# aidilayce/FollowMyHold

Hardware: AMD Instinct MI355X
Metric: guidance-steps/sec (512x512, 778+20k verts) (higher is better)
Workload: dtype f32; 1 GPU; configs[1]: 512x512 frame/GPU, 778-vert hand + 10242-vert/20480-face object, joint step (phase C); images_per_gpu=1, global_images=1, parallelism=image-sharded x1, steps_per_graph=1

## Files before the change

### followmyhold_amd/csrc/k_flexi.inc

```
#include "flexi_core.h"

constexpr int FX_ITEMS = 2048;

struct FlexiWs {
    uint8_t* cse;
    int32_t *npatch, *v_off, *ecross, *f_off, *bsum_v, *bsum_f;
    size_t total;
};
static FlexiWs carve_flexi(void* ws, int res) {
    const size_t G = (size_t)res + 1, C = (size_t)res * res * res, E = 3 * G * G * G;
    const size_t nbv = (C + FX_ITEMS - 1) / FX_ITEMS, nbf = (E + FX_ITEMS - 1) / FX_ITEMS;
    char* p = (char*)ws;
    Carve cv;
    FlexiWs w;
    w.cse = (uint8_t*)(p + cv.take(C));
    w.npatch = (int32_t*)(p + cv.take(C * 4));
    w.v_off = (int32_t*)(p + cv.take(C * 4));
    w.ecross = (int32_t*)(p + cv.take(E * 4));
    w.f_off = (int32_t*)(p + cv.take(E * 4));
    w.bsum_v = (int32_t*)(p + cv.take((nbv + 1) * 4));
    w.bsum_f = (int32_t*)(p + cv.take((nbf + 1) * 4));
    w.total = cv.off;
    return w;
}

extern "C" size_t foho_flexi_workspace_bytes(int32_t res) {
    if (res < 1 || res > 1024) return 0;
    return carve_flexi(nullptr, res).total;
}

__global__ __launch_bounds__(256) void k_flexi_classify(const float* s, int res, uint8_t* cse, int32_t* npatch, int32_t* ecross) {
    const int G = res + 1;
    const size_t t = (size_t)blockIdx.x * 256 + threadIdx.x;
    const size_t C = (size_t)res * res * res, G3 = (size_t)G * G * G;
    if (t < C) {
        const int k = (int)(t % res), j = (int)((t / res) % res), i = (int)(t / ((size_t)res * res));
        const unsigned code = flexi_cube_code(s, res, i, j, k);
        cse[t] = (uint8_t)code;
        npatch[t] = c_flexi_npatch[code];
    }
    if (t < 3 * G3) {
        const int axis = (int)(t / G3);
        const size_t r = t % G3;
        const int k = (int)(r % G), j = (int)((r / G) % G), i = (int)(r / ((size_t)G * G));
        const int di = axis == 0, dj = axis == 1, dk = axis == 2;
        int flag = 0;
        const bool along = (di ? i : (dj ? j : k)) < res;
        const bool t1 = di ? (j >= 1 && j <= res - 1) : (i >= 1 && i <= res - 1);
        const bool t2 = dk ? (j >= 1 && j <= res - 1) : (k >= 1 && k <= res - 1);
        if (along && t1 && t2) {
            const float sa = s[r], sb = s[((size_t)(i + di) * G + (j + dj)) * G + (k + dk)];
            flag = ((sa < 0.0f) != (sb < 0.0f)) ? 1 : 0;
        }
        ecross[t] = flag;
    }
}

__global__ __launch_bounds__(256) void k_scan_sums(const int32_t* in, size_t n, int32_t* bsum) {
    __shared__ int s_w[4];
    const size_t base = (size_t)blockIdx.x * FX_ITEMS + (size_t)threadIdx.x * 8;
    int v = 0;
#pragma unroll
    for (int q = 0; q < 8; q++) v += (base + q < n) ? in[base + q] : 0;
    const unsigned w = wave_sum((unsigned)v);
    if (lane_id() == 0) s_w[wave_id()] = (int)w;
    __syncthreads();
    if (threadIdx.x == 0) bsum[blockIdx.x] = (s_w[0] + s_w[1]) + (s_w[2] + s_w[3]);
}
__global__ __launch_bounds__(256) void k_scan_bsums(int32_t* bsum, int nb, int32_t* total) {
    __shared__ int s_w[4];
    __shared__ int s_carry;
    if (threadIdx.x == 0) s_carry = 0;
    __syncthreads();
    for (int base = 0; base < nb; base += 256) {
        const int i = base + threadIdx.x;
        const int v = (i < nb) ? bsum[i] : 0;
        const unsigned incl = wave_incl_scan((unsigned)v);
        if (lane_id() == 63) s_w[wave_id()] = (int)incl;
        __syncthreads();
        int off = s_carry;
        for (int w = 0; w < wave_id(); w++) off += s_w[w];
        if (i < nb) bsum[i] = off + (int)incl - v;
        __syncthreads();
        if (threadIdx.x == 0) s_carry += (s_w[0] + s_w[1]) + (s_w[2] + s_w[3]);
        __syncthreads();
    }
    if (threadIdx.x == 0) {
        bsum[nb] = s_carry;
        *total = s_carry;
    }
}
__global__ __launch_bounds__(256) void k_scan_apply(const int32_t* in, size_t n, const int32_t* bsum, int32_t* out) {
    __shared__ int s_w[4];
    const size_t base = (size_t)blockIdx.x * FX_ITEMS + (size_t)threadIdx.x * 8;
    int v[8], sum = 0;
#pragma unroll
    for (int q = 0; q < 8; q++) {
        v[q] = (base + q < n) ? in[base + q] : 0;
        sum += v[q];
    }
    const unsigned incl = wave_incl_scan((unsigned)sum);
    if (lane_id() == 63) s_w[wave_id()] = (int)incl;
    __syncthreads();
    int off = bsum[blockIdx.x] + (int)incl - sum;
    for (int w = 0; w < wave_id(); w++) off += s_w[w];
#pragma unroll
    for (int q = 0; q < 8; q++) {
        if (base + q < n) out[base + q] = off;
        off += v[q];
    }
}

struct Scan2 {
    const int32_t* in[2];
    size_t n[2];
    int32_t* bsum[2];
    int32_t* out[2];
    int nb[2];
};
__global__ __launch_bounds__(256) void k_scan2_sums(Scan2 a) {
    __shared__ int s_w[4];
    const int which = ((int)blockIdx.x < a.nb[0]) ? 0 : 1;
    const int blk = which ? blockIdx.x - a.nb[0] : blockIdx.x;
    const int32_t* in = which ? a.in[1] : a.in[0];
    const size_t n = which ? a.n[1] : a.n[0];
    const size_t base = (size_t)blk * FX_ITEMS + (size_t)threadIdx.x * 8;
    int v = 0;
#pragma unroll
    for (int q = 0; q < 8; q++) v += (base + q < n) ? in[base + q] : 0;
    const unsigned w = wave_sum((unsigned)v);
    if (lane_id() == 0) s_w[wave_id()] = (int)w;
    __syncthreads();
    if (threadIdx.x == 0) (which ? a.bsum[1] : a.bsum[0])[blk] = (s_w[0] + s_w[1]) + (s_w[2] + s_w[3]);
}
__device__ __forceinline__ int block_prefix(const int32_t* bsum, int blk, int* s_w) {
    int v = 0;
    for (int i = threadIdx.x; i < blk; i += 256) v += bsum[i];
    const unsigned w = wave_sum((unsigned)v);
    __syncthreads();
    if (lane_id() == 0) s_w[wave_id()] = (int)w;
    __syncthreads();
    const int r = (s_w[0] + s_w[1]) + (s_w[2] + s_w[3]);
    __syncthreads();
    return r;
}
__global__ __launch_bounds__(256) void k_scan2_apply(Scan2 a, int32_t* counts) {
    __shared__ int s_w[4];
    const int which = ((int)blockIdx.x < a.nb[0]) ? 0 : 1;
    const int blk = which ? blockIdx.x - a.nb[0] : blockIdx.x;
    const int32_t* in = which ? a.in[1] : a.in[0];
    const int32_t* bsum = which ? a.bsum[1] : a.bsum[0];
    int32_t* out = which ? a.out[1] : a.out[0];
    const size_t n = which ? a.n[1] : a.n[0];
    const size_t base = (size_t)blk * FX_ITEMS + (size_t)threadIdx.x * 8;
    int v[8], sum = 0;
#pragma unroll
    for (int q = 0; q < 8; q++) {
        v[q] = (base + q < n) ? in[base + q] : 0;
        sum += v[q];
    }
    const int prefix = block_prefix(bsum, blk, s_w);
    const unsigned incl = wave_incl_scan((unsigned)sum);
    if (lane_id() == 63) s_w[wave_id()] = (int)incl;
    __syncthreads();
    int off = prefix + (int)incl - sum;
    for (int w = 0; w < wave_id(); w++) off += s_w[w];
#pragma unroll
    for (int q = 0; q < 8; q++) {
        if (base + q < n) out[base + q] = off;
        off += v[q];
    }
    if (counts && blk == (which ? a.nb[1] : a.nb[0]) - 1 && threadIdx.x == 255) {
        if (which == 0) {
            counts[0] = off;
            counts[2] = 0;
        } else {
            counts[1] = 2 * off;
        }
    }
}
__global__ __launch_bounds__(256) void k_scan_apply_p(const int32_t* in, size_t n, const int32_t* bsum, int32_t* out) {
    __shared__ int s_w[4];
    const size_t base = (size_t)blockIdx.x * FX_ITEMS + (size_t)threadIdx.x * 8;
    int v[8], sum = 0;
#pragma unroll
    for (int q = 0; q < 8; q++) {
        v[q] = (base + q < n) ? in[base + q] : 0;
        sum += v[q];
    }
    const int prefix = block_prefix(bsum, (int)blockIdx.x, s_w);
    const unsigned incl = wave_incl_scan((unsigned)sum);
    if (lane_id() == 63) s_w[wave_id()] = (int)incl;
    __syncthreads();
    int off = prefix + (int)incl - sum;
    for (int w = 0; w < wave_id(); w++) off += s_w[w];
#pragma unroll
    for (int q = 0; q < 8; q++) {
        if (base + q < n) out[base + q] = off;
        off += v[q];
    }
}

__device__ __forceinline__ void flexi_corners(const float* x, const float* s, int res, size_t t, float* sc, float* xc) {
    const int G = res + 1;
    const int k = (int)(t % res), j = (int)((t / res) % res), i = (int)(t / ((size_t)res * res));
#pragma unroll
    for (int c = 0; c < 8; c++) {
        const size_t gi = ((size_t)(i + (c & 1)) * G + (j + ((c >> 1) & 1))) * G + (k + (c >> 2));
        sc[c] = s[gi];
        for (int q = 0; q < 3; q++) xc[3 * c + q] = x[3 * gi + q];
    }
}

__device__ __forceinline__ void flexi_verts_role(size_t t, const float* x, const float* s, int res, const uint8_t* cse, const int32_t* npatch,
                                                 const int32_t* v_off, float* verts, float* ldev, int cap, int32_t* counts) {
    if (t >= (size_t)res * res * res) return;
    const int np = npatch[t];
    if (np == 0) return;
    const int base = v_off[t];
    if (base + np > cap) {
        atomicOr(&counts[2], 1);
        return;
    }
    const unsigned code = cse[t];
    float sc[8], xc[24];
    flexi_corners(x, s, res, t, sc, xc);
    for (int p = 0; p < np; p++) flexi_dual_vertex(code, p, sc, xc, verts + 3 * (size_t)(base + p), ldev ? ldev + (base + p) : nullptr);
}

__device__ __forceinline__ void flexi_faces_role(size_t t, const float* s, int res, const uint8_t* cse, const int32_t* v_off,
                                                 const int32_t* ecross, const int32_t* f_off, int64_t* faces, int cap, int32_t* counts) {
    const int G = res + 1;
    const size_t G3 = (size_t)G * G * G;
    if (t >= 3 * G3 || !ecross[t]) return;
    const int qd = f_off[t];
    if (2 * qd + 2 > cap) {
        atomicOr(&counts[2], 2);
        return;
    }
    const int axis = (int)(t / G3);
    const size_t r = t % G3;
    const int k = (int)(r % G), j = (int)((r / G) % G), i = (int)(r / ((size_t)G * G));
    int64_t q[4];
#pragma unroll
    for (int c = 0; c < 4; c++) {
        const int ci = i + c_flexi_ring[axis][c][0], cj = j + c_flexi_ring[axis][c][1], ck = k + c_flexi_ring[axis][c][2];
        const size_t cid = ((size_t)ci * res + cj) * res + ck;
        q[c] = (int64_t)v_off[cid] + c_flexi_edge_patch[cse[cid]][c_flexi_ring[axis][c][3]];
    }
    flexi_quad(q, s[r] < 0.0f, faces + 6 * (size_t)qd);
}

__global__ __launch_bounds__(256) void k_flexi_emit(const float* x, const float* s, int res, const uint8_t* cse, const int32_t* npatch,
                                                    const int32_t* v_off, const int32_t* ecross, const int32_t* f_off, float* verts,
                                                    float* ldev, int verts_cap, int64_t* faces, int faces_cap, int32_t* counts, int nvb) {
    if ((int)blockIdx.x < nvb)
        flexi_verts_role((size_t)blockIdx.x * 256 + threadIdx.x, x, s, res, cse, npatch, v_off, verts, ldev, verts_cap, counts);
    else
        flexi_faces_role((size_t)(blockIdx.x - nvb) * 256 + threadIdx.x, s, res, cse, v_off, ecross, f_off, faces, faces_cap, counts);
}

extern "C" int foho_flexi_fwd(const float* x, const float* s, int32_t res, float* verts, int32_t verts_cap, int64_t* faces,
                              int32_t faces_cap, float* l_dev, int32_t* counts, void* workspace, size_t workspace_bytes,
                              void* stream_) {
    if (!x || !s || !verts || !faces || !counts || res < 1 || res > 1024 || verts_cap < 0 || faces_cap < 0) {
        foho_set_error("foho_flexi_fwd: bad argument");
        return FOHO_ERR_BAD_ARG;
    }
    const FlexiWs w = carve_flexi(workspace, res);
    if (!workspace || workspace_bytes < w.total) {
        foho_set_error("foho_flexi_fwd: workspace too small (query foho_flexi_workspace_bytes)");
        return FOHO_ERR_WORKSPACE;
    }
    hipStream_t stream = (hipStream_t)stream_;
    const size_t G = (size_t)res + 1, C = (size_t)res * res * res, E = 3 * G * G * G;
    const int nbv = (int)((C + FX_ITEMS - 1) / FX_ITEMS), nbf = (int)((E + FX_ITEMS - 1) / FX_ITEMS);
    hipLaunchKernelGGL(k_flexi_classify, dim3((unsigned)((E + 255) / 256)), dim3(256), 0, stream, s, res, w.cse, w.npatch, w.ecross);
    CHECK_LAUNCH("k_flexi_classify");
    Scan2 sc;
    sc.in[0] = w.npatch, sc.in[1] = w.ecross;
    sc.n[0] = C, sc.n[1] = E;
    sc.bsum[0] = w.bsum_v, sc.bsum[1] = w.bsum_f;
    sc.out[0] = w.v_off, sc.out[1] = w.f_off;
    sc.nb[0] = nbv, sc.nb[1] = nbf;
    hipLaunchKernelGGL(k_scan2_sums, dim3(nbv + nbf), dim3(256), 0, stream, sc);
    CHECK_LAUNCH("k_scan2_sums");
    hipLaunchKernelGGL(k_scan2_apply, dim3(nbv + nbf), dim3(256), 0, stream, sc, counts);
    CHECK_LAUNCH("k_scan2_apply");
    const int nvb = (int)((C + 255) / 256);
    hipLaunchKernelGGL(k_flexi_emit, dim3((unsigned)(nvb + (E + 255) / 256)), dim3(256), 0, stream, x, s, res, w.cse, w.npatch, w.v_off,
                       w.ecross, w.f_off, verts, l_dev, verts_cap, faces, faces_cap, counts, nvb);
    CHECK_LAUNCH("k_flexi_emit");
    return FOHO_OK;
}

__global__ __launch_bounds__(256) void k_flexi_bwd(const float* x, const float* s, int res, const uint8_t* cse, const int32_t* npatch,
                                                   const int32_t* v_off, const float* gverts, int n_verts, float* gs, float* gx) {
    const size_t t = (size_t)blockIdx.x * 256 + threadIdx.x;
    if (t >= (size_t)res * res * res) return;
    const int np = npatch[t];
    if (np == 0) return;
    const int base = v_off[t];
    if (base + np > n_verts) return;
    const int G = res + 1;
    const int k = (int)(t % res), j = (int)((t / res) % res), i = (int)(t / ((size_t)res * res));
    FLEXI_EDGE_TABLES
    const unsigned code = cse[t];
    float sc[8], xc[24];
    flexi_corners(x, s, res, t, sc, xc);
    for (int p = 0; p < np; p++) {
        float cnt = 0.f;
#pragma unroll
        for (int e = 0; e < 12; e++) cnt += (c_flexi_edge_patch[code][e] == p) ? 1.0f : 0.0f;
        float g[3];
        for (int q = 0; q < 3; q++) g[q] = gverts[3 * (size_t)(base + p) + q] / cnt;
#pragma unroll
        for (int e = 0; e < 12; e++) {
            if (c_flexi_edge_patch[code][e] != p) continue;
            const int a = fx_ea[e], b = fx_eb[e];
            const size_t ga = ((size_t)(i + (a & 1)) * G + (j + ((a >> 1) & 1))) * G + (k + (a >> 2));
            const size_t gb = ((size_t)(i + (b & 1)) * G + (j + ((b >> 1) & 1))) * G + (k + (b >> 2));
            const float D = sc[b] - sc[a];
            float dot = 0.f;
            for (int q = 0; q < 3; q++) dot += g[q] * (xc[3 * a + q] - xc[3 * b + q]);
            const float wa = sc[b] / D, wb = -sc[a] / D;
            atomicAdd(&gs[ga], dot * (wa / D));
            atomicAdd(&gs[gb], dot * (wb / D));
            if (gx) {
                for (int q = 0; q < 3; q++) {
                    atomicAdd(&gx[3 * ga + q], g[q] * wa);
                    atomicAdd(&gx[3 * gb + q], g[q] * wb);
                }
            }
        }
    }
}

extern "C" int foho_flexi_bwd(const float* x, const float* s, int32_t res, const float* grad_verts, int32_t n_verts, float* grad_s,
                              float* grad_x, const void* workspace, size_t workspace_bytes, void* stream_) {
    if (!x || !s || !grad_verts || !grad_s || res < 1 || res > 1024 || n_verts < 0) {
        foho_set_error("foho_flexi_bwd: bad argument");
        return FOHO_ERR_BAD_ARG;
    }
    const FlexiWs w = carve_flexi(const_cast<void*>(workspace), res);
    if (!workspace || workspace_bytes < w.total) {
        foho_set_error("foho_flexi_bwd: workspace too small");
        return FOHO_ERR_WORKSPACE;
    }
    hipStream_t stream = (hipStream_t)stream_;
    const size_t C = (size_t)res * res * res;
    hipLaunchKernelGGL(k_flexi_bwd, dim3((unsigned)((C + 255) / 256)), dim3(256), 0, stream, x, s, res, w.cse, w.npatch, w.v_off, grad_verts,
                       n_verts, grad_s, grad_x);
    CHECK_LAUNCH("k_flexi_bwd");
    return FOHO_OK;
}
```

### followmyhold_amd/csrc/k_object.inc

```

__global__ __launch_bounds__(256) void k_object_adopt(Ctx c, foho_image* img_rw, int32_t* faces_rw, const int32_t* counts,
                                                      const int64_t* obj_faces, int verts_cap, int faces_cap, int32_t* cnt) {
    const int b = blockIdx.y;
    const int v_off = img_rw[b].v_off, Vh = img_rw[b].Vh, f_off = img_rw[b].f_off, Fh = img_rw[b].Fh;
    int nv = counts[3 * b], nf = counts[3 * b + 1];
    const bool over = counts[3 * b + 2] != 0 || nv < 0 || nf < 0 || nv > verts_cap || nf > faces_cap;
    const bool odd = !over && (nf & 1);
    const bool bad = over || odd;
    if (bad) nv = nf = 0;
    const int64_t* src = obj_faces + (size_t)b * faces_cap * 3;
    int32_t* dst = faces_rw + 3 * (size_t)(f_off + Fh);
    const int shift = v_off + Vh;
    for (int j = blockIdx.x * 256 + threadIdx.x; j < 3 * nf; j += gridDim.x * 256) {
        const int v = (int32_t)src[j] + shift;
        dst[j] = v;
        atomicAdd(&cnt[v], 1);
    }
    const int32_t* hf = faces_rw + 3 * (size_t)f_off;
    for (int j = blockIdx.x * 256 + threadIdx.x; j < 3 * Fh; j += gridDim.x * 256) atomicAdd(&cnt[hf[j]], 1);
    if (blockIdx.x == 0 && threadIdx.x == 0) {
        img_rw[b].Vo = nv;
        img_rw[b].Fo = nf;
        img_rw[b].n_edges = 3 * nf / 2;
        if (bad) atomicOr(&c.flags[b], over ? 16 : 32);
        else if (nv == 0 || nf == 0) atomicOr(&c.flags[b], 64);
        for (int m = 0; m < 2; m++)
            for (int a = 0; a < 3; a++) c.mesh_info[2 * b + m].kmin_inv[a] = c.mesh_info[2 * b + m].kmax[a] = 0ull;
    }
}

__global__ __launch_bounds__(256) void k_object_fill(Ctx c, BboxCfg bc, int fgrid, const int32_t* inc_off, int32_t* cursor,
                                                     int32_t* inc_tmp) {
    if ((int)blockIdx.x >= fgrid) return bbox_role(c, bc, (int)blockIdx.x - fgrid, (int)blockIdx.y);
    const foho_image im = c.img[blockIdx.y];
    const int t = blockIdx.x * 256 + threadIdx.x;
    if (t >= 3 * (im.Fh + im.Fo)) return;
    const int v = c.faces[3 * (size_t)im.f_off + t], face = im.f_off + t / 3, corner = t % 3;
    inc_tmp[inc_off[v] + atomicAdd(&cursor[v], 1)] = (face << 2) | corner;
}

constexpr int TOPO_LDS_STRIDE = TOPO_MAXVAL + 1;
constexpr int TOPO_FAST = 16;
__global__ __launch_bounds__(64) void k_topo_finish_b(const int32_t* faces, int Vtot, int Fkey, const uint8_t* obj_flag,
                                                      const int32_t* inc_off, const int32_t* inc_tmp, int32_t* inc_fc,
                                                      int32_t* nbr_idx, unsigned long long* pair_v, const foho_image* img, int B, int32_t* flags,
                                                      int32_t* cnt, int32_t* cursor) {
    __shared__ int s_e[64 * TOPO_LDS_STRIDE], s_d[64 * TOPO_LDS_STRIDE], s_p[64 * TOPO_LDS_STRIDE];
    const int v = blockIdx.x * 64 + threadIdx.x;
    if (v >= Vtot) return;
    const int e0 = inc_off[v], n = inc_off[v + 1] - e0;
    cnt[v] = 0;
    cursor[v] = 0;
    if (n <= 0) return;
    int bad = 0;
    if (n > TOPO_MAXVAL) {
        bad = 1;
    } else if (n <= TOPO_FAST) {
        int x[TOPO_FAST], f[TOPO_FAST][3];
#pragma unroll
        for (int u = 0; u < TOPO_FAST; u++) x[u] = inc_tmp[e0 + min(u, n - 1)];
#pragma unroll
        for (int u = 0; u < TOPO_FAST; u++)
            for (int k = 0; k < 3; k++) f[u][k] = faces[3 * (size_t)(x[u] >> 2) + k];
        unsigned key[TOPO_FAST];
        int d[TOPO_FAST], pv[TOPO_FAST];
#pragma unroll
        for (int u = 0; u < TOPO_FAST; u++) {
            const int corner = x[u] & 3;
            key[u] = (u < n) ? (((unsigned)corner << 28) | (unsigned)(x[u] >> 2)) : 0xffffffffu;
            d[u] = (u < n) ? ((corner == 0) ? f[u][1] : ((corner == 1) ? f[u][2] : f[u][0])) : 0x7fffffff;
            pv[u] = (corner == 0) ? f[u][2] : ((corner == 1) ? f[u][0] : f[u][1]);
        }
        const bool check = obj_flag[v] != 0;
#pragma unroll
        for (int u = 0; u < TOPO_FAST; u++) {
            int rk = 0, rd = 0, dup = 0, found = 0;
#pragma unroll
            for (int j = 0; j < TOPO_FAST; j++) {
                rk += (key[j] < key[u]) ? 1 : 0;
                rd += (d[j] < d[u] || (d[j] == d[u] && j < u)) ? 1 : 0;
                dup |= (j < u && d[j] == d[u]) ? 1 : 0;
                found |= (d[j] == pv[u]) ? 1 : 0;
            }
            if (u < n) {
                inc_fc[e0 + rk] = x[u];
                pair_v[e0 + rk] = pack_pair(f[u][0], f[u][1], f[u][2], x[u] & 3);
                nbr_idx[e0 + rd] = d[u];
                if (check) bad |= dup | (found ^ 1);
            }
        }
    } else {
        int* e = s_e + threadIdx.x * TOPO_LDS_STRIDE;
        int* d = s_d + threadIdx.x * TOPO_LDS_STRIDE;
        int* pv = s_p + threadIdx.x * TOPO_LDS_STRIDE;
        for (int base = 0; base < n; base += 8) {
            int x[8];
#pragma unroll
            for (int u = 0; u < 8; u++) x[u] = inc_tmp[e0 + min(base + u, n - 1)];
#pragma unroll
            for (int u = 0; u < 8; u++)
                if (base + u < n) e[base + u] = x[u];
        }
        for (int a = 1; a < n; a++) {
            const int x = e[a];
            const long long kx = (long long)(x & 3) * Fkey + (x >> 2);
            int b2 = a - 1;
            while (b2 >= 0) {
                const int y = e[b2];
                if (((long long)(y & 3) * Fkey + (y >> 2)) <= kx) break;
                e[b2 + 1] = y;
                b2--;
            }
            e[b2 + 1] = x;
        }
        for (int base = 0; base < n; base += 8) {
            int x[8], f[8][3];
#pragma unroll
            for (int u = 0; u < 8; u++) x[u] = e[min(base + u, n - 1)];
#pragma unroll
            for (int u = 0; u < 8; u++)
                for (int k = 0; k < 3; k++) f[u][k] = faces[3 * (size_t)(x[u] >> 2) + k];
#pragma unroll
            for (int u = 0; u < 8; u++) {
                if (base + u >= n) break;
                const int corner = x[u] & 3;
                inc_fc[e0 + base + u] = x[u];
                pair_v[e0 + base + u] = pack_pair(f[u][0], f[u][1], f[u][2], corner);
                d[base + u] = (corner == 0) ? f[u][1] : ((corner == 1) ? f[u][2] : f[u][0]);
                pv[base + u] = (corner == 0) ? f[u][2] : ((corner == 1) ? f[u][0] : f[u][1]);
            }
        }
        for (int a = 1; a < n; a++) {
            const int x = d[a];
            int b2 = a - 1;
            while (b2 >= 0) {
                const int y = d[b2];
                if (y <= x) break;
                d[b2 + 1] = y;
                b2--;
            }
            d[b2 + 1] = x;
        }
        for (int q = 0; q < n; q++) nbr_idx[e0 + q] = d[q];
        if (obj_flag[v]) {
            for (int q = 1; q < n; q++) bad |= (d[q] == d[q - 1]);
            for (int q = 0; q < n && !bad; q++) {
                const int p = pv[q];
                bool found = false;
                for (int r = 0; r < n; r++) found = found || (d[r] == p);
                bad = !found;
            }
        }
    }
    if (bad)
        for (int b = 0; b < B; b++)
            if (v >= img[b].v_off && v < img[b].v_off + img[b].Vh + img[b].Vo) atomicOr(&flags[b], 32);
}

extern "C" size_t foho_object_workspace_bytes(int32_t Vtot, int32_t Ftot) {
    if (Vtot < 1 || Ftot < 1) return 0;
    const size_t n = (size_t)Vtot + 1, nb = (n + FX_ITEMS - 1) / FX_ITEMS;
    return 2 * al(n * 4) + al((nb + 1) * 4) + al((size_t)Ftot * 3 * 4);
}

extern "C" int foho_object_update(const foho_step_desc* desc, const int32_t* counts, const int64_t* obj_faces,
                                  int32_t faces_cap, const uint8_t* obj_flag, void* workspace, size_t workspace_bytes,
                                  void* stream_) {
    if (!desc || !counts || !obj_faces || !obj_flag || faces_cap < 0) {
        foho_set_error("foho_object_update: null argument");
        return FOHO_ERR_BAD_ARG;
    }
    const foho_dims& d = desc->dims;
    if (d.B < 1 || d.Vtot < 1 || d.Ftot < 1 || d.Ftot >= (1 << 28) || d.Fmax < 1 || faces_cap > d.Fo_max) {
        foho_set_error("foho_object_update: bad dims (Vo_max / Fo_max are the per-image object capacities)");
        return FOHO_ERR_BAD_ARG;
    }
    if (!pair_limits_ok(d)) {
        foho_set_error("foho_object_update: more than 4194304 vertex slots per batch or 524287 per image is not supported (pair table)");
        return FOHO_ERR_BAD_ARG;
    }
    const WS w = make_ws(d);
    if (!desc->workspace || desc->workspace_bytes < w.total || !workspace ||
        workspace_bytes < foho_object_workspace_bytes(d.Vtot, d.Ftot)) {
        foho_set_error("foho_object_update: workspace too small (foho_step_workspace_bytes / foho_object_workspace_bytes)");
        return FOHO_ERR_WORKSPACE;
    }
    hipStream_t stream = (hipStream_t)stream_;
    Ctx c = make_ctx(*desc, w);
    const size_t n = (size_t)d.Vtot + 1;
    const int nb = (int)((n + FX_ITEMS - 1) / FX_ITEMS);
    char* p = (char*)workspace;
    int32_t* cnt = (int32_t*)p;
    int32_t* cursor = (int32_t*)(p + al(n * 4));
    int32_t* bsum = (int32_t*)(p + 2 * al(n * 4));
    int32_t* inc_tmp = (int32_t*)(p + 2 * al(n * 4) + al(((size_t)nb + 1) * 4));
    const int fgrid = cdiv(3 * d.Fmax, 256);
    hipLaunchKernelGGL(k_object_adopt, dim3(std::max(1, std::min(fgrid, 128)), d.B), dim3(256), 0, stream, c,
                       const_cast<foho_image*>(desc->images), const_cast<int32_t*>(desc->faces), counts, obj_faces, d.Vo_max, faces_cap, cnt);
    CHECK_LAUNCH("k_object_adopt");
    hipLaunchKernelGGL(k_scan_sums, dim3(nb), dim3(256), 0, stream, cnt, n, bsum);
    CHECK_LAUNCH("k_scan_sums");
    hipLaunchKernelGGL(k_scan_apply_p, dim3(nb), dim3(256), 0, stream, cnt, n, bsum, const_cast<int32_t*>(desc->inc_off));
    CHECK_LAUNCH("k_scan_apply_p");
    BboxCfg bc;
    bc.nbh = cdiv(d.Vh_max > 0 ? d.Vh_max : 1, 256);
    bc.nbo = cdiv(d.Vo_max > 0 ? d.Vo_max : 1, 256);
    hipLaunchKernelGGL(k_object_fill, dim3(fgrid + bc.nbh + bc.nbo, d.B), dim3(256), 0, stream, c, bc, fgrid, desc->inc_off, cursor, inc_tmp);
    CHECK_LAUNCH("k_object_fill");
    hipLaunchKernelGGL(k_topo_finish_b, dim3(cdiv(d.Vtot, 64)), dim3(64), 0, stream, desc->faces, d.Vtot, d.Ftot, obj_flag, desc->inc_off,
                       inc_tmp, const_cast<int32_t*>(desc->inc_fc), const_cast<int32_t*>(desc->nbr_idx), c.pair_v, desc->images, d.B,
                       desc->flags, cnt, cursor);
    CHECK_LAUNCH("k_topo_finish_b");
    return FOHO_OK;
}
```

### followmyhold_amd/csrc/k_vertex.inc

```

__device__ __forceinline__ void load_moge(const Ctx& c, const foho_image& im, int mesh, int gi, float* v) {
    const float x = c.verts_in[3 * gi], y = c.verts_in[3 * gi + 1], z = c.verts_in[3 * gi + 2];
    if (mesh == 0) {
        v[0] = x;
        v[1] = y;
        v[2] = z;
    } else {
        const float* M = im.T_h2m;
        v[0] = ((x * M[0] + y * M[1]) + z * M[2]) + M[3];
        v[1] = ((x * M[4] + y * M[5]) + z * M[6]) + M[7];
        v[2] = ((x * M[8] + y * M[9]) + z * M[10]) + M[11];
    }
}

struct BboxCfg {
    int nbh, nbo;
};
__global__ __launch_bounds__(64) void k_bbox_clear(MeshInfo* mi, int n) {
    const int i = blockIdx.x * 64 + threadIdx.x;
    if (i < n)
        for (int a = 0; a < 3; a++) mi[i].kmin_inv[a] = mi[i].kmax[a] = 0ull;
}
__device__ void bbox_role(const Ctx& c, const BboxCfg& cfg, int bx, int b) {
    __shared__ unsigned long long s_k[6][4];
    const foho_image im = c.img[b];
    const int mesh = (bx < cfg.nbh) ? 0 : 1;
    const int blk = mesh ? (bx - cfg.nbh) : bx;
    const int n = mesh ? im.Vo : im.Vh;
    if (blk * 256 >= n) return;
    const int base = im.v_off + (mesh ? im.Vh : 0);
    const int i = blk * 256 + threadIdx.x;
    unsigned long long k[6] = {0ull, 0ull, 0ull, 0ull, 0ull, 0ull};
    if (i < n) {
        float v[3];
        load_moge(c, im, mesh, base + i, v);
        for (int a = 0; a < 3; a++) {
            const unsigned long long o = (unsigned long long)f2ord(v[a]) << 32;
            k[a] = ~(o | (unsigned)i);
            k[3 + a] = o | (unsigned)(~(unsigned)i);
        }
    }
    for (int a = 0; a < 6; a++) {
        unsigned long long x = k[a];
#pragma unroll
        for (int o = 32; o > 0; o >>= 1) {
            const unsigned long long y = __shfl_down(x, o, 64);
            x = (y > x) ? y : x;
        }
        if (lane_id() == 0) s_k[a][wave_id()] = x;
    }
    __syncthreads();
    if (threadIdx.x < 6) {
        unsigned long long x = s_k[threadIdx.x][0];
        for (int w = 1; w < 4; w++) x = (s_k[threadIdx.x][w] > x) ? s_k[threadIdx.x][w] : x;
        MeshInfo* mi = &c.mesh_info[b * 2 + mesh];
        unsigned long long* dst = (threadIdx.x < 3) ? &mi->kmin_inv[threadIdx.x] : &mi->kmax[threadIdx.x - 3];
        atomicMax(dst, x);
    }
}
__global__ __launch_bounds__(256) void k_bbox(Ctx c, BboxCfg cfg) { bbox_role(c, cfg, (int)blockIdx.x, (int)blockIdx.y); }

__global__ __launch_bounds__(256) void k_pair_table(Ctx c, int n) {
    const int e = blockIdx.x * 256 + threadIdx.x;
    if (e >= n) return;
    const int fc = c.inc_fc[e], f = fc >> 2;
    c.pair_v[e] = pack_pair(c.faces[3 * f], c.faces[3 * f + 1], c.faces[3 * f + 2], fc & 3);
}

__device__ void world_boxes(const Ctx& c, const foho_image& im, int b, float* s_box) {
    if (wave_id() == 0) {
        float v[12];
        for (int mesh = 0; mesh < 2; mesh++) {
            for (int a = 0; a < 3; a++) {
                v[6 * mesh + a] = INFINITY;
                v[6 * mesh + 3 + a] = -INFINITY;
            }
            const int nb = ((mesh ? im.Vo : im.Vh) + 255) / 256;
            for (int blk = lane_id(); blk < nb; blk += 64) {
                const float* row = c.xf_part + (((size_t)b * 2 + mesh) * VERT_BLOCKS_MAX + blk) * 8;
                for (int a = 0; a < 3; a++) {
                    v[6 * mesh + a] = fminf(v[6 * mesh + a], row[a]);
                    v[6 * mesh + 3 + a] = fmaxf(v[6 * mesh + 3 + a], row[3 + a]);
                }
            }
        }
        for (int q = 0; q < 12; q++) {
            const float x = ((q % 6) < 3) ? wave_min(v[q]) : wave_max(v[q]);
            if (lane_id() == 0) s_box[q] = x;
        }
    }
    __syncthreads();
}

struct Stage2Cfg {
    int nA, nC, nD, nE, nI;
    int lean_h, lean_o, lean_i;
    int nIh, if_h, if_o;
    float* acc;
    int knn_chunks;
    int hand_order_valid;
    int nRh, nRo, rf_h, rf_o;
    foho_render_cfg render[2];
    int n_renders, sil_bits;
    bool vn_hand, vn_obj;
    int dbg;
    float blur_radius, sqrt_blur, sigma;
    float full_t;
    float w_edge, w_verts, w_contact, contact_margin;
};

__device__ void role_normals(const Ctx& c, const foho_image& im, const Stage2Cfg& cfg, int blk) {
    const int i = blk * 256 + threadIdx.x;
    if (i >= im.Vh + im.Vo) return;
    if (!((i < im.Vh) ? cfg.vn_hand : cfg.vn_obj)) return;
    const int gv = im.v_off + i;
    float acc[3] = {0.f, 0.f, 0.f};
    const int e0 = c.inc_off[gv], e1 = c.inc_off[gv + 1];
    for (int base = e0; base < e1; base += 8) {
        int fid[8], vi[8][3];
        float P[8][9];
#pragma unroll
        for (int u = 0; u < 8; u++) fid[u] = c.inc_fc[min(base + u, e1 - 1)] >> 2;
#pragma unroll
        for (int u = 0; u < 8; u++)
            for (int k = 0; k < 3; k++) vi[u][k] = c.faces[3 * fid[u] + k];
#pragma unroll
        for (int u = 0; u < 8; u++)
            for (int k = 0; k < 3; k++)
                for (int q = 0; q < 3; q++) P[u][3 * k + q] = c.world[3 * vi[u][k] + q];
#pragma unroll
        for (int u = 0; u < 8; u++) {
            if (base + u >= e1) break;
            float A[3], Bv[3], n[3];
            for (int k = 0; k < 3; k++) {
                A[k] = P[u][6 + k] - P[u][3 + k];
                Bv[k] = P[u][k] - P[u][3 + k];
            }
            cross3(A, Bv, n);
            acc[0] += n[0];
            acc[1] += n[1];
            acc[2] += n[2];
        }
    }
    const float nrm = sqrtf((acc[0] * acc[0] + acc[1] * acc[1]) + acc[2] * acc[2]);
    const float den = fmaxf(nrm, 1e-6f);
    for (int k = 0; k < 3; k++) c.vn[3 * gv + k] = acc[k] / den;
    const float inv = 1.0f / den;
    const bool reg = nrm > 1e-6f;
    reinterpret_cast<float4*>(c.vn_raw)[gv] = make_float4(reg ? acc[0] * inv : 0.0f, reg ? acc[1] * inv : 0.0f, reg ? acc[2] * inv : 0.0f, inv);
}

template <bool P2>
__device__ __forceinline__ void ndc_to_pix_range_t(float lo, float hi, const PixAxis& ax, int& p0, int& p1) {
    const int S1 = ax.S1;
    const float off = ax.offset;
    auto centre = [&](int i) {
        const float num = ax.range * (float)i + ax.offset;
        return -ax.offset + (P2 ? num * ax.inv_s1 : num / ax.s1);
    };
    const float nlo = (lo + off) * ax.s1 - off, nhi = (hi + off) * ax.s1 - off;
    float flo = P2 ? nlo * ax.inv_range : nlo / ax.range;
    float fhi = P2 ? nhi * ax.inv_range : nhi / ax.range;
    flo = fminf(fmaxf(flo, -2.0f), ax.s1 + 1.0f);
    fhi = fminf(fmaxf(fhi, -2.0f), ax.s1 + 1.0f);
    int i0 = max(0, (int)ceilf(flo)), i1 = min(S1 - 1, (int)floorf(fhi));
    const int e0 = min(i0, S1), e1 = max(i1, -1);
    bool a[4], b[4];
#pragma unroll
    for (int k = 0; k < 4; k++) {
        const int ia = e0 - 2 + k, ib = e1 - 1 + k;
        a[k] = (ia >= S1) | ((ia >= 0) & (centre(ia) >= lo));
        b[k] = (ib < 0) | ((ib < S1) & (centre(ib) <= hi));
    }
    if (a[0] | !a[3] | !b[0] | b[3]) {
        i0 = 0;
        while (i0 < S1 && centre(i0) < lo) i0++;
        i1 = S1 - 1;
        while (i1 >= 0 && centre(i1) > hi) i1--;
    } else {
        i0 = a[1] ? e0 - 1 : (a[2] ? e0 : e0 + 1);
        i1 = b[2] ? e1 + 1 : (b[1] ? e1 : e1 - 1);
    }
    p0 = S1 - 1 - i1;
    p1 = S1 - 1 - i0;
}
__device__ __forceinline__ void ndc_to_pix_range(float lo, float hi, const PixAxis& ax, int& p0, int& p1) {
    if (ax.pow2 && ax.range_pow2) ndc_to_pix_range_t<true>(lo, hi, ax, p0, p1);
    else ndc_to_pix_range_t<false>(lo, hi, ax, p0, p1);
}
__device__ __forceinline__ void ndc_to_pix_range(float lo, float hi, int S1, int S2, int& p0, int& p1) {
    ndc_to_pix_range(lo, hi, pix_axis(S1, S2), p0, p1);
}

constexpr int KNN_Q = 64, KNN_CH = 1024, KNN_GRP = 8;
constexpr int KNN_ST = 512;
typedef float knn_f2 __attribute__((ext_vector_type(2)));
__device__ void role_knn(const Ctx& c, const foho_image& im, const Stage2Cfg& cfg, int b, int blk, unsigned char* lds) {
    const int wv = wave_id(), lane = lane_id(), tid = threadIdx.x;
    const int nqb = cfg.nC / cfg.knn_chunks;
    const int oc = blk / nqb, qb = blk - oc * nqb;
    float* s_x = reinterpret_cast<float*>(lds);
    float* s_y = s_x + KNN_ST;
    float* s_z = s_y + KNN_ST;
    unsigned long long* s_best = reinterpret_cast<unsigned long long*>(lds + KNN_ST * 12);
    const int ob = im.v_off + im.Vh, j0 = oc * KNN_CH;
    const bool work = qb * KNN_Q < im.Vh && j0 < im.Vo;
    const int slot = qb * KNN_Q + lane;
// ... 216 lines not shown
```

Before: 16090 guidance-steps/s.

## Fuse scan block sums into classify and build incidence lists during adopt

The flexi classify kernel now processes FX_ITEMS elements per 1024-thread block and emits per-block sums for both the patch counts and the edge-crossing flags, so the separate scan-sums launch is removed. In the object update, incidence entries are written into a vertex-strided temporary table during adopt via the atomic counter's return value, which removes the cursor array and the fill kernel. A single-block scan with bbox work fused into the same launch replaces the two-kernel scan when the vertex count fits. The cost is a larger workspace (Vtot*TOPO_MAXVAL), a scattered strided write layout, and more launched blocks for adopt.

```diff
diff --git a/followmyhold_amd/csrc/k_flexi.inc b/followmyhold_amd/csrc/k_flexi.inc
--- a/followmyhold_amd/csrc/k_flexi.inc
+++ b/followmyhold_amd/csrc/k_flexi.inc
@@ -29,30 +29,72 @@
     return carve_flexi(nullptr, res).total;
 }
 
-__global__ __launch_bounds__(256) void k_flexi_classify(const float* s, int res, uint8_t* cse, int32_t* npatch, int32_t* ecross) {
-    const int G = res + 1;
-    const size_t t = (size_t)blockIdx.x * 256 + threadIdx.x;
-    const size_t C = (size_t)res * res * res, G3 = (size_t)G * G * G;
-    if (t < C) {
-        const int k = (int)(t % res), j = (int)((t / res) % res), i = (int)(t / ((size_t)res * res));
-        const unsigned code = flexi_cube_code(s, res, i, j, k);
-        cse[t] = (uint8_t)code;
-        npatch[t] = c_flexi_npatch[code];
-    }
-    if (t < 3 * G3) {
+constexpr int CL_THREADS = 1024, CL_Q = FX_ITEMS / CL_THREADS;
+__global__ __launch_bounds__(CL_THREADS) void k_flexi_classify(const float* s, int res, uint8_t* cse, int32_t* npatch, int32_t* ecross,
+                                                               int32_t* bsum_v, int32_t* bsum_f, int nbv) {
+    __shared__ int s_w[2][CL_THREADS / 64];
+    const unsigned G = (unsigned)res + 1, R = (unsigned)res;
+    const unsigned C = R * R * R, G3 = G * G * G, E = 3 * G3;
+    const unsigned base = blockIdx.x * (unsigned)FX_ITEMS + threadIdx.x;
+    int nv = 0, nf = 0;
+    if ((int)blockIdx.x < nbv) {
+        unsigned code[CL_Q];
+        int np[CL_Q];
+#pragma unroll
+        for (int q = 0; q < CL_Q; q++) {
+            const unsigned t = min(base + (unsigned)q * CL_THREADS, C - 1);
+            code[q] = flexi_cube_code(s, res, (int)(t / (R * R)), (int)((t / R) % R), (int)(t % R));
+        }
+#pragma unroll
+        for (int q = 0; q < CL_Q; q++) np[q] = c_flexi_npatch[code[q]];
+#pragma unroll
+        for (int q = 0; q < CL_Q; q++) {
+            const unsigned t = base + (unsigned)q * CL_THREADS;
+            if (t < C) {
+                cse[t] = (uint8_t)code[q];
+                npatch[t] = np[q];
+                nv += np[q];
+            }
+        }
+    }
+    float sa[CL_Q], sb[CL_Q];
+    bool ok[CL_Q];
+#pragma unroll
+    for (int q = 0; q < CL_Q; q++) {
+        const unsigned t = min(base + (unsigned)q * CL_THREADS, E - 1);
         const int axis = (int)(t / G3);
-        const size_t r = t % G3;
-        const int k = (int)(r % G), j = (int)((r / G) % G), i = (int)(r / ((size_t)G * G));
+        const unsigned r = t % G3;
+        const int k = (int)(r % G), j = (int)((r / G) % G), i = (int)(r / (G * G));
         const int di = axis == 0, dj = axis == 1, dk = axis == 2;
-        int flag = 0;
         const bool along = (di ? i : (dj ? j : k)) < res;
         const bool t1 = di ? (j >= 1 && j <= res - 1) : (i >= 1 && i <= res - 1);
         const bool t2 = dk ? (j >= 1 && j <= res - 1) : (k >= 1 && k <= res - 1);
-        if (along && t1 && t2) {
-            const float sa = s[r], sb = s[((size_t)(i + di) * G + (j + dj)) * G + (k + dk)];
-            flag = ((sa < 0.0f) != (sb < 0.0f)) ? 1 : 0;
-        }
-        ecross[t] = flag;
+        ok[q] = along && t1 && t2;
+        sa[q] = s[r];
+        sb[q] = s[((size_t)min(i + di, res) * G + min(j + dj, res)) * G + min(k + dk, res)];
+    }
+#pragma unroll
+    for (int q = 0; q < CL_Q; q++) {
+        const unsigned t = base + (unsigned)q * CL_THREADS;
+        const int flag = (ok[q] && ((sa[q] < 0.0f) != (sb[q] < 0.0f))) ? 1 : 0;
+        if (t < E) {
+            ecross[t] = flag;
+            nf += flag;
+        }
+    }
+    const unsigned wv = wave_sum((unsigned)nv), wf = wave_sum((unsigned)nf);
+    if (lane_id() == 0) {
+        s_w[0][wave_id()] = (int)wv;
+        s_w[1][wave_id()] = (int)wf;
+    }
+    __syncthreads();
+    if (wave_id() == 0) {
+        const int l = lane_id();
+        const unsigned bv = wave_sum((unsigned)(l < CL_THREADS / 64 ? s_w[0][l] : 0)), bf = wave_sum((unsigned)(l < CL_THREADS / 64 ? s_w[1][l] : 0));
+        if (l == 0) {
+            if ((int)blockIdx.x < nbv) bsum_v[blockIdx.x] = (int)bv;
+            bsum_f[blockIdx.x] = (int)bf;
+        }
     }
 }
 
@@ -118,21 +160,6 @@
     int32_t* out[2];
     int nb[2];
 };
-__global__ __launch_bounds__(256) void k_scan2_sums(Scan2 a) {
-    __shared__ int s_w[4];
-    const int which = ((int)blockIdx.x < a.nb[0]) ? 0 : 1;
-    const int blk = which ? blockIdx.x - a.nb[0] : blockIdx.x;
-    const int32_t* in = which ? a.in[1] : a.in[0];
-    const size_t n = which ? a.n[1] : a.n[0];
-    const size_t base = (size_t)blk * FX_ITEMS + (size_t)threadIdx.x * 8;
-    int v = 0;
-#pragma unroll
-    for (int q = 0; q < 8; q++) v += (base + q < n) ? in[base + q] : 0;
-    const unsigned w = wave_sum((unsigned)v);
-    if (lane_id() == 0) s_w[wave_id()] = (int)w;
-    __syncthreads();
-    if (threadIdx.x == 0) (which ? a.bsum[1] : a.bsum[0])[blk] = (s_w[0] + s_w[1]) + (s_w[2] + s_w[3]);
-}
 __device__ __forceinline__ int block_prefix(const int32_t* bsum, int blk, int* s_w) {
     int v = 0;
     for (int i = threadIdx.x; i < blk; i += 256) v += bsum[i];
@@ -179,28 +206,6 @@
         }
     }
 }
-__global__ __launch_bounds__(256) void k_scan_apply_p(const int32_t* in, size_t n, const int32_t* bsum, int32_t* out) {
-    __shared__ int s_w[4];
-    const size_t base = (size_t)blockIdx.x * FX_ITEMS + (size_t)threadIdx.x * 8;
-    int v[8], sum = 0;
-#pragma unroll
-    for (int q = 0; q < 8; q++) {
-        v[q] = (base + q < n) ? in[base + q] : 0;
-        sum += v[q];
-    }
-    const int prefix = block_prefix(bsum, (int)blockIdx.x, s_w);
-    const unsigned incl = wave_incl_scan((unsigned)sum);
-    if (lane_id() == 63) s_w[wave_id()] = (int)incl;
-    __syncthreads();
-    int off = prefix + (int)incl - sum;
-    for (int w = 0; w < wave_id(); w++) off += s_w[w];
-#pragma unroll
-    for (int q = 0; q < 8; q++) {
-        if (base + q < n) out[base + q] = off;
-        off += v[q];
-    }
-}
-
 __device__ __forceinline__ void flexi_corners(const float* x, const float* s, int res, size_t t, float* sc, float* xc) {
     const int G = res + 1;
     const int k = (int)(t % res), j = (int)((t / res) % res), i = (int)(t / ((size_t)res * res));
@@ -275,7 +280,7 @@
     hipStream_t stream = (hipStream_t)stream_;
     const size_t G = (size_t)res + 1, C = (size_t)res * res * res, E = 3 * G * G * G;
     const int nbv = (int)((C + FX_ITEMS - 1) / FX_ITEMS), nbf = (int)((E + FX_ITEMS - 1) / FX_ITEMS);
-    hipLaunchKernelGGL(k_flexi_classify, dim3((unsigned)((E + 255) / 256)), dim3(256), 0, stream, s, res, w.cse, w.npatch, w.ecross);
+    hipLaunchKernelGGL(k_flexi_classify, dim3(nbf), dim3(CL_THREADS), 0, stream, s, res, w.cse, w.npatch, w.ecross, w.bsum_v, w.bsum_f, nbv);
     CHECK_LAUNCH("k_flexi_classify");
     Scan2 sc;
     sc.in[0] = w.npatch, sc.in[1] = w.ecross;
@@ -283,8 +288,6 @@
     sc.bsum[0] = w.bsum_v, sc.bsum[1] = w.bsum_f;
     sc.out[0] = w.v_off, sc.out[1] = w.f_off;
     sc.nb[0] = nbv, sc.nb[1] = nbf;
-    hipLaunchKernelGGL(k_scan2_sums, dim3(nbv + nbf), dim3(256), 0, stream, sc);
-    CHECK_LAUNCH("k_scan2_sums");
     hipLaunchKernelGGL(k_scan2_apply, dim3(nbv + nbf), dim3(256), 0, stream, sc, counts);
     CHECK_LAUNCH("k_scan2_apply");
     const int nvb = (int)((C + 255) / 256);
diff --git a/followmyhold_amd/csrc/k_object.inc b/followmyhold_amd/csrc/k_object.inc
--- a/followmyhold_amd/csrc/k_object.inc
+++ b/followmyhold_amd/csrc/k_object.inc
@@ -1,6 +1,7 @@
 
 __global__ __launch_bounds__(256) void k_object_adopt(Ctx c, foho_image* img_rw, int32_t* faces_rw, const int32_t* counts,
-                                                      const int64_t* obj_faces, int verts_cap, int faces_cap, int32_t* cnt) {
+                                                      const int64_t* obj_faces, int verts_cap, int faces_cap, int32_t* cnt,
+                                                      int32_t* inc_tmp) {
     const int b = blockIdx.y;
     const int v_off = img_rw[b].v_off, Vh = img_rw[b].Vh, f_off = img_rw[b].f_off, Fh = img_rw[b].Fh;
     int nv = counts[3 * b], nf = counts[3 * b + 1];
@@ -14,10 +15,15 @@
     for (int j = blockIdx.x * 256 + threadIdx.x; j < 3 * nf; j += gridDim.x * 256) {
         const int v = (int32_t)src[j] + shift;
         dst[j] = v;
-        atomicAdd(&cnt[v], 1);
+        const int old = atomicAdd(&cnt[v], 1);
+        if (old < TOPO_MAXVAL) inc_tmp[(size_t)old * c.d.Vtot + v] = ((f_off + Fh + j / 3) << 2) | (j % 3);
     }
     const int32_t* hf = faces_rw + 3 * (size_t)f_off;
-    for (int j = blockIdx.x * 256 + threadIdx.x; j < 3 * Fh; j += gridDim.x * 256) atomicAdd(&cnt[hf[j]], 1);
+    for (int j = blockIdx.x * 256 + threadIdx.x; j < 3 * Fh; j += gridDim.x * 256) {
+        const int v = hf[j];
+        const int old = atomicAdd(&cnt[v], 1);
+        if (old < TOPO_MAXVAL) inc_tmp[(size_t)old * c.d.Vtot + v] = ((f_off + j / 3) << 2) | (j % 3);
+    }
     if (blockIdx.x == 0 && threadIdx.x == 0) {
         img_rw[b].Vo = nv;
         img_rw[b].Fo = nf;
@@ -29,14 +35,90 @@
     }
 }
 
-__global__ __launch_bounds__(256) void k_object_fill(Ctx c, BboxCfg bc, int fgrid, const int32_t* inc_off, int32_t* cursor,
-                                                     int32_t* inc_tmp) {
-    if ((int)blockIdx.x >= fgrid) return bbox_role(c, bc, (int)blockIdx.x - fgrid, (int)blockIdx.y);
-    const foho_image im = c.img[blockIdx.y];
-    const int t = blockIdx.x * 256 + threadIdx.x;
-    if (t >= 3 * (im.Fh + im.Fo)) return;
-    const int v = c.faces[3 * (size_t)im.f_off + t], face = im.f_off + t / 3, corner = t % 3;
-    inc_tmp[inc_off[v] + atomicAdd(&cursor[v], 1)] = (face << 2) | corner;
+constexpr int SCAN1_THREADS = 1024, SCAN1_CHUNKS = 12;
+constexpr int SCAN1_REACH = SCAN1_THREADS * 4 * SCAN1_CHUNKS;
+__device__ __forceinline__ void scan1_role(const int32_t* in, int n, int32_t* out) {
+    __shared__ int s_w[SCAN1_CHUNKS * (SCAN1_THREADS / 64)];
+    constexpr int NW = SCAN1_THREADS / 64;
+    int v[SCAN1_CHUNKS][4], sum[SCAN1_CHUNKS], incl[SCAN1_CHUNKS];
+#pragma unroll
+    for (int c = 0; c < SCAN1_CHUNKS; c++) {
+        const int i = c * (SCAN1_THREADS * 4) + 4 * (int)threadIdx.x;
+        if (i + 3 < n) {
+            const int4 x = *(const int4*)(in + i);
+            v[c][0] = x.x, v[c][1] = x.y, v[c][2] = x.z, v[c][3] = x.w;
+        } else {
+#pragma unroll
+            for (int q = 0; q < 4; q++) v[c][q] = (i + q < n) ? in[i + q] : 0;
+        }
+        sum[c] = (v[c][0] + v[c][1]) + (v[c][2] + v[c][3]);
+    }
+#pragma unroll
+    for (int c = 0; c < SCAN1_CHUNKS; c++) {
+        incl[c] = (int)wave_incl_scan((unsigned)sum[c]);
+        if (lane_id() == 63) s_w[c * NW + wave_id()] = incl[c];
+    }
+    __syncthreads();
+    static_assert(NW == 16 && SCAN1_CHUNKS % 4 == 0, "entry c * 16 + wave sits in group c / 4");
+    constexpr int EPL = SCAN1_CHUNKS * NW / 64;
+    int ex[EPL], carry = 0;
+#pragma unroll
+    for (int e = 0; e < EPL; e++) {
+        const int a = s_w[64 * e + lane_id()];
+        const int in_e = (int)wave_incl_scan((unsigned)a);
+        ex[e] = carry + in_e - a;
+        carry += __builtin_amdgcn_readlane(in_e, 63);
+    }
+#pragma unroll
+    for (int c = 0; c < SCAN1_CHUNKS; c++) {
+        const int idx = c * NW + wave_id();
+        const int pre = __shfl(ex[c / 4], idx & 63, 64);
+        int off = pre + incl[c] - sum[c];
+        const int i = c * (SCAN1_THREADS * 4) + 4 * (int)threadIdx.x;
+        int4 o;
+        o.x = off, off += v[c][0];
+        o.y = off, off += v[c][1];
+        o.z = off, off += v[c][2];
+        o.w = off;
+        if (i + 3 < n) {
+            *(int4*)(out + i) = o;
+        } else {
+            if (i < n) out[i] = o.x;
+            if (i + 1 < n) out[i + 1] = o.y;
+            if (i + 2 < n) out[i + 2] = o.z;
+        }
+    }
+}
+__global__ __launch_bounds__(SCAN1_THREADS) void k_object_scan1(Ctx c, BboxCfg bc, const int32_t* cnt, int n, int32_t* inc_off) {
+    if (blockIdx.x == 0) return scan1_role(cnt, n, inc_off);
+    const int per = bc.nbh + bc.nbo, j = (int)blockIdx.x - 1;
+    bbox_role<SCAN1_THREADS>(c, bc, j % per, j / per);
+}
+__global__ __launch_bounds__(256) void k_scan_apply_p(Ctx c, BboxCfg bc, int nb, const int32_t* in, size_t n, const int32_t* bsum,
+                                                      int32_t* out) {
+    if ((int)blockIdx.x >= nb) {
+        const int per = bc.nbh + bc.nbo, j = (int)blockIdx.x - nb;
+        return bbox_role(c, bc, j % per, j / per);
+    }
+    __shared__ int s_w[4];
+    const size_t base = (size_t)blockIdx.x * FX_ITEMS + (size_t)threadIdx.x * 8;
+    int v[8], sum = 0;
+#pragma unroll
+    for (int q = 0; q < 8; q++) {
+        v[q] = (base + q < n) ? in[base + q] : 0;
+        sum += v[q];
+    }
+    const int prefix = block_prefix(bsum, (int)blockIdx.x, s_w);
+    const unsigned incl = wave_incl_scan((unsigned)sum);
+    if (lane_id() == 63) s_w[wave_id()] = (int)incl;
+    __syncthreads();
+    int off = prefix + (int)incl - sum;
+    for (int w = 0; w < wave_id(); w++) off += s_w[w];
+#pragma unroll
+    for (int q = 0; q < 8; q++) {
+        if (base + q < n) out[base + q] = off;
+        off += v[q];
+    }
 }
 
 constexpr int TOPO_LDS_STRIDE = TOPO_MAXVAL + 1;
@@ -44,13 +126,13 @@
 __global__ __launch_bounds__(64) void k_topo_finish_b(const int32_t* faces, int Vtot, int Fkey, const uint8_t* obj_flag,
                                                       const int32_t* inc_off, const int32_t* inc_tmp, int32_t* inc_fc,
                                                       int32_t* nbr_idx, unsigned long long* pair_v, const foho_image* img, int B, int32_t* flags,
-                                                      int32_t* cnt, int32_t* cursor) {
+                                                      int32_t* cnt) {
     __shared__ int s_e[64 * TOPO_LDS_STRIDE], s_d[64 * TOPO_LDS_STRIDE], s_p[64 * TOPO_LDS_STRIDE];
     const int v = blockIdx.x * 64 + threadIdx.x;
     if (v >= Vtot) return;
     const int e0 = inc_off[v], n = inc_off[v + 1] - e0;
     cnt[v] = 0;
-    cursor[v] = 0;
+    const int32_t* lst = inc_tmp + v;
     if (n <= 0) return;
     int bad = 0;
     if (n > TOPO_MAXVAL) {
@@ -58,7 +140,7 @@
     } else if (n <= TOPO_FAST) {
         int x[TOPO_FAST], f[TOPO_FAST][3];
 #pragma unroll
-        for (int u = 0; u < TOPO_FAST; u++) x[u] = inc_tmp[e0 + min(u, n - 1)];
+        for (int u = 0; u < TOPO_FAST; u++) x[u] = lst[(size_t)min(u, n - 1) * Vtot];
 #pragma unroll
         for (int u = 0; u < TOPO_FAST; u++)
             for (int k = 0; k < 3; k++) f[u][k] = faces[3 * (size_t)(x[u] >> 2) + k];
@@ -96,7 +178,7 @@
         for (int base = 0; base < n; base += 8) {
             int x[8];
 #pragma unroll
-            for (int u = 0; u < 8; u++) x[u] = inc_tmp[e0 + min(base + u, n - 1)];
+            for (int u = 0; u < 8; u++) x[u] = lst[(size_t)min(base + u, n - 1) * Vtot];
 #pragma unroll
             for (int u = 0; u < 8; u++)
                 if (base + u < n) e[base + u] = x[u];
@@ -160,7 +242,7 @@
 extern "C" size_t foho_object_workspace_bytes(int32_t Vtot, int32_t Ftot) {
     if (Vtot < 1 || Ftot < 1) return 0;
     const size_t n = (size_t)Vtot + 1, nb = (n + FX_ITEMS - 1) / FX_ITEMS;
-    return 2 * al(n * 4) + al((nb + 1) * 4) + al((size_t)Ftot * 3 * 4);
+    return al(n * 4) + al((nb + 1) * 4) + al((size_t)Vtot * TOPO_MAXVAL * 4);
 }
 
 extern "C" int foho_object_update(const foho_step_desc* desc, const int32_t* counts, const int64_t* obj_faces,
@@ -191,25 +273,31 @@
     const int nb = (int)((n + FX_ITEMS - 1) / FX_ITEMS);
     char* p = (char*)workspace;
     int32_t* cnt = (int32_t*)p;
-    int32_t* cursor = (int32_t*)(p + al(n * 4));
-    int32_t* bsum = (int32_t*)(p + 2 * al(n * 4));
-    int32_t* inc_tmp = (int32_t*)(p + 2 * al(n * 4) + al(((size_t)nb + 1) * 4));
+    int32_t* bsum = (int32_t*)(p + al(n * 4));
+    int32_t* inc_tmp = (int32_t*)(p + al(n * 4) + al(((size_t)nb + 1) * 4));
+    int32_t* inc_off = const_cast<int32_t*>(desc->inc_off);
     const int fgrid = cdiv(3 * d.Fmax, 256);
-    hipLaunchKernelGGL(k_object_adopt, dim3(std::max(1, std::min(fgrid, 128)), d.B), dim3(256), 0, stream, c,
-                       const_cast<foho_image*>(desc->images), const_cast<int32_t*>(desc->faces), counts, obj_faces, d.Vo_max, faces_cap, cnt);
+    hipLaunchKernelGGL(k_object_adopt, dim3(std::max(1, fgrid), d.B), dim3(256), 0, stream, c,
+                       const_cast<foho_image*>(desc->images), const_cast<int32_t*>(desc->faces), counts, obj_faces, d.Vo_max, faces_cap, cnt,
+                       inc_tmp);
     CHECK_LAUNCH("k_object_adopt");
-    hipLaunchKernelGGL(k_scan_sums, dim3(nb), dim3(256), 0, stream, cnt, n, bsum);
-    CHECK_LAUNCH("k_scan_sums");
-    hipLaunchKernelGGL(k_scan_apply_p, dim3(nb), dim3(256), 0, stream, cnt, n, bsum, const_cast<int32_t*>(desc->inc_off));
-    CHECK_LAUNCH("k_scan_apply_p");
     BboxCfg bc;
-    bc.nbh = cdiv(d.Vh_max > 0 ? d.Vh_max : 1, 256);
-    bc.nbo = cdiv(d.Vo_max > 0 ? d.Vo_max : 1, 256);
-    hipLaunchKernelGGL(k_object_fill, dim3(fgrid + bc.nbh + bc.nbo, d.B), dim3(256), 0, stream, c, bc, fgrid, desc->inc_off, cursor, inc_tmp);
-    CHECK_LAUNCH("k_object_fill");
+    if (n <= (size_t)SCAN1_REACH && (((uintptr_t)cnt | (uintptr_t)inc_off) & 15) == 0) {
+        bc.nbh = cdiv(d.Vh_max > 0 ? d.Vh_max : 1, SCAN1_THREADS);
+        bc.nbo = cdiv(d.Vo_max > 0 ? d.Vo_max : 1, SCAN1_THREADS);
+        hipLaunchKernelGGL(k_object_scan1, dim3(1 + (bc.nbh + bc.nbo) * d.B), dim3(SCAN1_THREADS), 0, stream, c, bc, cnt, (int)n, inc_off);
+        CHECK_LAUNCH("k_object_scan1");
+    } else {
+        bc.nbh = cdiv(d.Vh_max > 0 ? d.Vh_max : 1, 256);
+        bc.nbo = cdiv(d.Vo_max > 0 ? d.Vo_max : 1, 256);
+        hipLaunchKernelGGL(k_scan_sums, dim3(nb), dim3(256), 0, stream, cnt, n, bsum);
+        CHECK_LAUNCH("k_scan_sums");
+        hipLaunchKernelGGL(k_scan_apply_p, dim3(nb + (bc.nbh + bc.nbo) * d.B), dim3(256), 0, stream, c, bc, nb, cnt, n, bsum, inc_off);
+        CHECK_LAUNCH("k_scan_apply_p");
+    }
     hipLaunchKernelGGL(k_topo_finish_b, dim3(cdiv(d.Vtot, 64)), dim3(64), 0, stream, desc->faces, d.Vtot, d.Ftot, obj_flag, desc->inc_off,
                        inc_tmp, const_cast<int32_t*>(desc->inc_fc), const_cast<int32_t*>(desc->nbr_idx), c.pair_v, desc->images, d.B,
-                       desc->flags, cnt, cursor);
+                       desc->flags, cnt);
     CHECK_LAUNCH("k_topo_finish_b");
     return FOHO_OK;
 }
diff --git a/followmyhold_amd/csrc/k_vertex.inc b/followmyhold_amd/csrc/k_vertex.inc
--- a/followmyhold_amd/csrc/k_vertex.inc
+++ b/followmyhold_amd/csrc/k_vertex.inc
@@ -21,15 +21,16 @@
     if (i < n)
         for (int a = 0; a < 3; a++) mi[i].kmin_inv[a] = mi[i].kmax[a] = 0ull;
 }
+template <int NT = 256>
 __device__ void bbox_role(const Ctx& c, const BboxCfg& cfg, int bx, int b) {
-    __shared__ unsigned long long s_k[6][4];
+    __shared__ unsigned long long s_k[6][NT / 64];
     const foho_image im = c.img[b];
     const int mesh = (bx < cfg.nbh) ? 0 : 1;
     const int blk = mesh ? (bx - cfg.nbh) : bx;
     const int n = mesh ? im.Vo : im.Vh;
-    if (blk * 256 >= n) return;
+    if (blk * NT >= n) return;
     const int base = im.v_off + (mesh ? im.Vh : 0);
-    const int i = blk * 256 + threadIdx.x;
+    const int i = blk * NT + threadIdx.x;
     unsigned long long k[6] = {0ull, 0ull, 0ull, 0ull, 0ull, 0ull};
     if (i < n) {
         float v[3];
@@ -52,7 +53,7 @@
     __syncthreads();
     if (threadIdx.x < 6) {
         unsigned long long x = s_k[threadIdx.x][0];
-        for (int w = 1; w < 4; w++) x = (s_k[threadIdx.x][w] > x) ? s_k[threadIdx.x][w] : x;
+        for (int w = 1; w < NT / 64; w++) x = (s_k[threadIdx.x][w] > x) ? s_k[threadIdx.x][w] : x;
         MeshInfo* mi = &c.mesh_info[b * 2 + mesh];
         unsigned long long* dst = (threadIdx.x < 3) ? &mi->kmin_inv[threadIdx.x] : &mi->kmax[threadIdx.x - 3];
         atomicMax(dst, x);
```

Result: no change. 16010 guidance-steps/s (-0.5%).
